# david8862/tf-keras-speech-commands

Hardware: AMD Instinct MI355X
Metric: 1 s@16 kHz clips/sec train-step, simple_cnn bs4096, 1/2/4/8 MI355X; eval top-1 (higher is better)
Workload: dtype f32; 1 GPU; configs[1]: simple_cnn train step = featurize(f32 1 s @16 kHz) + fwd + bwd + Adam, 36 logits (background + 35 words), batch 4096 per GPU; global_batch=4096, parallelism=dp1, gradient_exchange=none (one rank), rccl_ranks=0, library_build=546ca62dfe01

## Files before the change

### tf-keras-speech-commands_amd/csrc/kws_conv_group.h

```cpp
#pragma once

namespace kws {

constexpr int kGrThreads = 1024, kGrWaves = kGrThreads / 64;

template <int C, int G>
__device__ __forceinline__ void group_stats(float s, float ss, int ch, int grp, int lq, double *red, double *__restrict__ partial, int stride,
                                            double *__restrict__ acc = nullptr)
{
    double a = (double)s, q = (double)ss;
    a += __shfl_xor(a, 16, 64); a += __shfl_xor(a, 32, 64);
    q += __shfl_xor(q, 16, 64); q += __shfl_xor(q, 32, 64);
    if (lq == 0) { red[(grp * 2 + 0) * C + ch] = a; red[(grp * 2 + 1) * C + ch] = q; }
    __syncthreads();
    for (int i = threadIdx.x; i < 2 * C; i += kGrThreads) {
        const int which = i / C, n = i - which * C;
        double t = 0.0;
#pragma unroll
        for (int g2 = 0; g2 < G; ++g2) t += red[(g2 * 2 + which) * C + n];
        if (acc) acc_add(acc, 2 * C, i, t);
        else partial[((long)which * C + n) * stride + blockIdx.x] = t;
    }
}

// ... 139 lines not shown
        __shared__ __attribute__((aligned(16))) float cf3[2 * kFuC3];
        f32x4 sc, sh;
        if (g.in.acc) {
            bn_fwd_coef_prologue(g.in, kFuC3, cf3, cf3 + kFuC3);
            sc = *reinterpret_cast<const f32x4 *>(cf3 + 4 * (tid & 15)); sh = *reinterpret_cast<const f32x4 *>(cf3 + kFuC3 + 4 * (tid & 15));
        } else {
            sc = *reinterpret_cast<const f32x4 *>(g.sc3 + 4 * (tid & 15)); sh = *reinterpret_cast<const f32x4 *>(g.sh3 + 4 * (tid & 15));
        }
        for (int i = tid; i < kFuClips * PER; i += kGrThreads) {
            const int c = i / PER, r = i - c * PER, pos = r >> 4, u4 = r & 15;
            f32x4 v = {0.f, 0.f, 0.f, 0.f};
            if (b0 + c < g.B) {
                const f32x4 z = *reinterpret_cast<const f32x4 *>(g.z3 + ((long)(b0 + c) * PER + r) * 4);
#pragma unroll
                for (int e = 0; e < 4; ++e) v[e] = relu6f(fmaf(z[e], sc[e], sh[e]));
            }
            bf16x4 h, m, l;
            split_bf16(v, h, m, l);
            const int e0 = ((pos * kFuClips + c) * 8 + ((u4 >> 1) ^ ((c >> 1) & 7))) * 8 + (u4 & 1) * 4;
            *reinterpret_cast<bf16x4 *>(A3 + e0) = h;
            *reinterpret_cast<bf16x4 *>(A3 + kFuA3P + e0) = m;
            *reinterpret_cast<bf16x4 *>(A3 + 2 * kFuA3P + e0) = l;
        }
    }
    __syncthreads();
    f32x4 acc[NP];
#pragma unroll
    for (int q = 0; q < NP; ++q) acc[q] = (f32x4){0.f, 0.f, 0.f, 0.f};
#pragma unroll 1
    for (int ks3 = 0; ks3 < 18; ks3 += 3) {
#pragma unroll
        for (int d = 0; d < 3; ++d) {
            const int ks = ks3 + d;
            if (ks + 2 < 18) fu_load_b(g.f4, (long)(ks + 2) * 8 + ct, lane, b4[(d + 2) % 3]);
            const int tap = ks >> 1, chunk = ks & 1, kh = tap / 3, kw = tap - kh * 3;
            const int uo = ((4 * chunk + lq) ^ sw) * 8;
#pragma unroll
            for (int q = 0; q < NP; ++q) {
                const int pos = NP * grp + q, oh = pos / kFuW3, ow = pos - oh * kFuW3;
                const int ih = oh + kh - 1, iw = ow + kw - 1;
                if (ih >= 0 && ih < kFuH3 && iw >= 0 && iw < kFuW3) {
                    const __bf16 *row = A3 + ((ih * kFuW3 + iw) * kFuClips + li) * kFuC3 + uo;
                    bf16x8 a[3];
#pragma unroll
                    for (int p = 0; p < 3; ++p) a[p] = *reinterpret_cast<const bf16x8 *>(row + p * kFuA3P);
                    acc[q] = mfma_bf16x6(a, b4[d], acc[q]);
                }
            }
        }
    }
    const int ch = 16 * ct + li;
    float s = 0.f, ss = 0.f;
#pragma unroll
    for (int q = 0; q < NP; ++q) {
        const int pos = NP * grp + q;
#pragma unroll
        for (int r = 0; r < 4; ++r) {
            const int clip = 4 * lq + r;
            const float v = fmaxf(acc[q][r], 0.f);
            if (b0 + clip < g.B) g.z4[((long)(b0 + clip) * (kFuH3 * kFuW3) + pos) * kFuC4 + ch] = v;
            s += v; ss = fmaf(v, v, ss);
        }
    }
    __syncthreads();
    group_stats<kFuC4, kGrWaves / 8>(s, ss, ch, grp, lq, reinterpret_cast<double *>(gr_lds), g.partial, g.stride, g.acc);
}

constexpr int kGrD4P = kFuH3 * kFuW3 * kFuClips * kFuC4;
struct GroupDgrad4Args { const __bf16 *dz[3], *fw[3]; const float *z3, *coef; float *g3; double *partial; int stride, B; double *acc; };

__global__ __launch_bounds__(kGrThreads, 1) void conv4_group_dgrad_kernel(GroupDgrad4Args g)
{
    extern __shared__ __attribute__((aligned(16))) float gr_lds[];
    __bf16 *D4 = reinterpret_cast<__bf16 *>(gr_lds);
    const int tid = threadIdx.x, lane = tid & 63, wave = __builtin_amdgcn_readfirstlane(tid >> 6), li = lane & 15, lq = lane >> 4;
    const int b0 = blockIdx.x * kFuClips;
    constexpr int NP = 12 / (kGrWaves / 4);
    const int ct = wave & 3, grp = wave >> 2;
    bf16x8 bw[3][3];
    fu_load_b(g.fw, ct, lane, bw[0]);
    fu_load_b(g.fw, 4 + ct, lane, bw[1]);
    {
        constexpr int PER = kFuH3 * kFuW3 * kFuC4 / 8;
        for (int i = tid; i < 3 * kFuClips * PER; i += kGrThreads) {
            const int p = i / (kFuClips * PER), r0 = i - p * (kFuClips * PER), c = r0 / PER, r = r0 - c * PER, pos = r >> 4, u = r & 15;
            bf16x8 v = {0, 0, 0, 0, 0, 0, 0, 0};
            if (b0 + c < g.B) v = *reinterpret_cast<const bf16x8 *>(g.dz[p] + ((long)(b0 + c) * PER + r) * 8);
            *reinterpret_cast<bf16x8 *>(D4 + p * kGrD4P + ((pos * kFuClips + c) * 16 + (u ^ (c & 15))) * 8) = v;
        }
    }
    __syncthreads();
    f32x4 acc[NP];
#pragma unroll
    for (int q = 0; q < NP; ++q) acc[q] = (f32x4){0.f, 0.f, 0.f, 0.f};
#pragma unroll 1
    for (int ks3 = 0; ks3 < 36; ks3 += 3) {
#pragma unroll
        for (int d = 0; d < 3; ++d) {
            const int ks = ks3 + d;
            if (ks + 2 < 36) fu_load_b(g.fw, (long)(ks + 2) * 4 + ct, lane, bw[(d + 2) % 3]);
            const int tap = ks >> 2, chunk = ks & 3, kh = tap / 3, kw = tap - kh * 3;
            const int uo = ((4 * chunk + lq) ^ li) * 8;
#pragma unroll
            for (int q = 0; q < NP; ++q) {
                const int pos = NP * grp + q, y = pos / kFuW3, x = pos - y * kFuW3;
                const int sy = y + 1 - kh, sx = x + 1 - kw;
                if (sy >= 0 && sy < kFuH3 && sx >= 0 && sx < kFuW3) {
                    const __bf16 *row = D4 + ((sy * kFuW3 + sx) * kFuClips + li) * kFuC4 + uo;
                    bf16x8 a[3];
#pragma unroll
                    for (int p = 0; p < 3; ++p) a[p] = *reinterpret_cast<const bf16x8 *>(row + p * kGrD4P);
                    acc[q] = mfma_bf16x6(a, bw[d], acc[q]);
                }
            }
        }
    }
    const int ch = 16 * ct + li;
    const float gsc = g.coef[ch], gsh = g.coef[kFuC3 + ch], gmean = g.coef[2 * kFuC3 + ch], ginv = g.coef[3 * kFuC3 + ch];
    float s = 0.f, ss = 0.f;
    float z3v[NP][4];
#pragma unroll
    for (int q = 0; q < NP; ++q)
#pragma unroll
        for (int r = 0; r < 4; ++r) {
            const int clip = 4 * lq + r;
            z3v[q][r] = b0 + clip < g.B ? g.z3[((long)(b0 + clip) * (kFuH3 * kFuW3) + NP * grp + q) * kFuC3 + ch] : 0.f;
        }
#pragma unroll
    for (int q = 0; q < NP; ++q) {
        const int pos = NP * grp + q;
#pragma unroll
        for (int r = 0; r < 4; ++r) {
            const int clip = 4 * lq + r;
            if (b0 + clip < g.B) {
                const long e = ((long)(b0 + clip) * (kFuH3 * kFuW3) + pos) * kFuC3 + ch;
                const float zv = z3v[q][r], yv = fmaf(zv, gsc, gsh);
                const float v = (yv > 0.f && yv < 6.f) ? acc[q][r] : 0.f;
                g.g3[e] = v;
                s += v; ss = fmaf(v, (zv - gmean) * ginv, ss);
            }
        }
    }
    __syncthreads();
    group_stats<kFuC3, kGrWaves / 4>(s, ss, ch, grp, lq, reinterpret_cast<double *>(gr_lds), g.partial, g.stride, g.acc);
}

struct GroupDgrad3Args { const float *dz3; const __bf16 *fw[3]; float *da2; int B; const float *zmax2, *coef2; double *acc; };

__global__ __launch_bounds__(kGrThreads, 1) void conv3_group_dgrad_kernel(GroupDgrad3Args g)
{
    extern __shared__ __attribute__((aligned(16))) float gr_lds[];
    __bf16 *D3 = reinterpret_cast<__bf16 *>(gr_lds);
    const int tid = threadIdx.x, lane = tid & 63, wave = __builtin_amdgcn_readfirstlane(tid >> 6), li = lane & 15, lq = lane >> 4;
    const int b0 = blockIdx.x * kFuClips;
    const int sw = (li >> 1) & 7;
    constexpr int NPOS = kFuH2 * kFuW2, NG = kGrWaves / 2, NP = (NPOS + NG - 1) / NG;
    const int ct = wave & 1, grp = wave >> 1;
    bf16x8 bw[3][3];
    fu_load_b(g.fw, ct, lane, bw[0]);
    fu_load_b(g.fw, 2 + ct, lane, bw[1]);
    {
        constexpr int PER = kFuH3 * kFuW3 * kFuC3 / 4;
        for (int i = tid; i < kFuClips * PER; i += kGrThreads) {
            const int c = i / PER, r = i - c * PER, pos = r >> 4, u4 = r & 15;
            f32x4 v = {0.f, 0.f, 0.f, 0.f};
            if (b0 + c < g.B) v = *reinterpret_cast<const f32x4 *>(g.dz3 + ((long)(b0 + c) * PER + r) * 4);
            bf16x4 h, m, l;
            split_bf16(v, h, m, l);
            const int e0 = ((pos * kFuClips + c) * 8 + ((u4 >> 1) ^ ((c >> 1) & 7))) * 8 + (u4 & 1) * 4;
            *reinterpret_cast<bf16x4 *>(D3 + e0) = h;
            *reinterpret_cast<bf16x4 *>(D3 + kFuA3P + e0) = m;
            *reinterpret_cast<bf16x4 *>(D3 + 2 * kFuA3P + e0) = l;
        }
    }
    __syncthreads();
    f32x4 acc[NP];
#pragma unroll
    for (int q = 0; q < NP; ++q) acc[q] = (f32x4){0.f, 0.f, 0.f, 0.f};
#pragma unroll 1
    for (int ks3 = 0; ks3 < 18; ks3 += 3) {
#pragma unroll
        for (int d = 0; d < 3; ++d) {
            const int ks = ks3 + d;
            if (ks + 2 < 18) fu_load_b(g.fw, (long)(ks + 2) * 2 + ct, lane, bw[(d + 2) % 3]);
            const int tap = ks >> 1, chunk = ks & 1, kh = tap / 3, kw = tap - kh * 3;
            const int uo = ((4 * chunk + lq) ^ sw) * 8;
#pragma unroll
            for (int q = 0; q < NP; ++q) {
                const int pos = NP * grp + q, y = pos / kFuW2, x = pos - y * kFuW2;
                const int sy = y + 1 - kh, sx = x + 1 - kw;
                if (pos < NPOS && sy >= 0 && sx >= 0 && !((sy | sx) & 1) && (sy >> 1) < kFuH3 && (sx >> 1) < kFuW3) {
                    const __bf16 *row = D3 + (((sy >> 1) * kFuW3 + (sx >> 1)) * kFuClips + li) * kFuC3 + uo;
                    bf16x8 a[3];
#pragma unroll
                    for (int p = 0; p < 3; ++p) a[p] = *reinterpret_cast<const bf16x8 *>(row + p * kFuA3P);
                    acc[q] = mfma_bf16x6(a, bw[d], acc[q]);
                }
            }
        }
    }
    const int ch = 16 * ct + li;
    if (g.acc) {
        const float gsc = g.coef2[ch], gsh = g.coef2[kFuC2 + ch], gmean = g.coef2[2 * kFuC2 + ch], ginv = g.coef2[3 * kFuC2 + ch];
        float s = 0.f, sx = 0.f;
        float za[NP][4];
#pragma unroll
        for (int q = 0; q < NP; ++q)
#pragma unroll
            for (int r = 0; r < 4; ++r) {
                const int pos = NP * grp + q, clip = 4 * lq + r;
// ... 36 lines not shown
```

### tf-keras-speech-commands_amd/csrc/kws_dense_head.h

```cpp
#pragma once

namespace kws {

constexpr int kDhK = 128, kDhCP = 48, kDhCS = 50;
constexpr int kDhKS = kDhK + 8;

struct DenseHeadArgs {
    const float *a4;
    const __bf16 *fd[3], *fo[3];
    const float *db, *w2;
    float *d1, *dd1, *da4;
    float *dw2, *db2, *ddb;
    int B, C, flat;
    HeadFwdArgs fw;
    const float *zmax4 = nullptr, *coef4 = nullptr;
    double *acc4 = nullptr;
    float drop_rate = 0.f;
    uint32_t seed_lo = 0, seed_hi = 0;
    const float *z4 = nullptr;
    BnAccFwd in4{};
    float *a4w = nullptr, *zmax4w = nullptr;
    unsigned char *arg4w = nullptr;
    int H3 = 0, W3 = 0;
};

constexpr int kDhWaves = 8, kDhThreads = 64 * kDhWaves;
__global__ __launch_bounds__(kDhThreads) void dense_head_fused_kernel(DenseHeadArgs g)
{
    constexpr int NW = kDhWaves, NT = kDhThreads;
    static_assert(NW == 4 || NW == 8, "column tiles per wave below: 8 / NW Dense tiles, 24 / NW dW2 tiles");
    constexpr int DT = 8 / NW, WT = 24 / NW;
    extern __shared__ __attribute__((aligned(16))) float dh_lds[];
    const int RS4 = g.flat + 8;
    float *a4s = dh_lds;
    float *xs = a4s + 16 * RS4;
    float *dd = xs + 16 * kDhKS;
    float *ds = dd + 16 * kDhKS;
    float *ws = ds + 16 * kDhCS;
    const int tid = threadIdx.x, lane = tid & 63, wave = __builtin_amdgcn_readfirstlane(tid >> 6), li = lane & 15, lq = lane >> 4;
    const int b0 = blockIdx.x * 16, C = g.C, K = kDhK;
    const int nks = g.flat / 32;

    bf16x8 bcur[DT][3], bnext[DT][3];
#pragma unroll
    for (int t = 0; t < DT; ++t) fu_load_b(g.fd, DT * wave + t, lane, bcur[t]);
    constexpr int NW2 = kDhK * kDhCP / NT;
    static_assert(kDhK * kDhCP % NT == 0, "whole rounds");
    float w2v[NW2];
#pragma unroll
    for (int j = 0; j < NW2; ++j) { const int i = tid + j * NT, k = i / kDhCP, c = i - k * kDhCP; w2v[j] = c < C ? g.w2[(long)k * C + c] : 0.f; }
    __shared__ __attribute__((aligned(16))) float cf4[4 * kDhK];
    if (g.z4) {
        bn_fwd_coef_prologue(g.in4, kDhK, cf4, cf4 + kDhK, cf4 + 2 * kDhK, cf4 + 3 * kDhK);
        const int W4 = g.W3 / 2, nf4 = g.flat / 4;
        constexpr int NB = 2;
        for (int base = tid; base < 16 * nf4; base += NB * NT) {
            f32x4 z[NB][4];
#pragma unroll
            for (int k = 0; k < NB; ++k) {
                const int i = base + NT * k, r = i / nf4, u = i - r * nf4, win = u / (kDhK / 4), c0 = 4 * (u - win * (kDhK / 4));
                const int ph = win / W4, pw = win - ph * W4;
                const bool ok = i < 16 * nf4 && b0 + r < g.B;
                const float *zp = g.z4 + ((((long)(b0 + r) * g.H3 + 2 * ph) * g.W3 + 2 * pw) * kDhK + c0);
#pragma unroll
                for (int j = 0; j < 4; ++j)
                    z[k][j] = ok ? *reinterpret_cast<const f32x4 *>(zp + ((j >> 1) * g.W3 + (j & 1)) * kDhK) : (f32x4){0.f, 0.f, 0.f, 0.f};
            }
#pragma unroll
            for (int k = 0; k < NB; ++k) {
                const int i = base + NT * k, r = i / nf4, u = i - r * nf4, c0 = 4 * (u % (kDhK / 4));
                if (i >= 16 * nf4) continue;
                f32x4 v = {0.f, 0.f, 0.f, 0.f};
                if (b0 + r < g.B) {
                    const f32x4 sc = *reinterpret_cast<const f32x4 *>(cf4 + c0), sh = *reinterpret_cast<const f32x4 *>(cf4 + kDhK + c0);
                    const long o = (long)(b0 + r) * g.flat + 4 * u;
                    f32x4 zm;
                    unsigned am = 0u;
#pragma unroll
                    for (int e = 0; e < 4; ++e) {
                        const float y0 = fmaf(z[k][0][e], sc[e], sh[e]), y1 = fmaf(z[k][1][e], sc[e], sh[e]);
                        const float y2 = fmaf(z[k][2][e], sc[e], sh[e]), y3 = fmaf(z[k][3][e], sc[e], sh[e]);
                        float a = relu6f(fmaxf(fmaxf(y0, y1), fmaxf(y2, y3)));
                        unsigned arg = 0u;
                        float best = relu6f(y0), zz = z[k][0][e];
                        const float v1 = relu6f(y1), v2 = relu6f(y2), v3 = relu6f(y3);
                        if (v1 > best) { best = v1; arg = 1u; zz = z[k][1][e]; }
                        if (v2 > best) { best = v2; arg = 2u; zz = z[k][2][e]; }
                        if (v3 > best) { arg = 3u; zz = z[k][3][e]; }
                        zm[e] = zz;
                        am |= arg << (8 * e);
                        if (g.drop_rate > 0.f) a = dropout_keep(g.seed_lo, g.seed_hi, (uint32_t)(o + e), g.drop_rate) ? a / (1.f - g.drop_rate) : 0.f;
                        v[e] = a;
                    }
                    *reinterpret_cast<f32x4 *>(g.a4w + o) = v;
                    *reinterpret_cast<f32x4 *>(g.zmax4w + o) = zm;
                    *reinterpret_cast<unsigned *>(g.arg4w + o) = am;
                }
                *reinterpret_cast<f32x4 *>(a4s + r * RS4 + 4 * u) = v;
            }
        }
    } else
    for (int i = tid; i < 16 * (g.flat / 4); i += NT) {
        const int r = i / (g.flat / 4), u = i - r * (g.flat / 4);
        f32x4 v = {0.f, 0.f, 0.f, 0.f};
        if (b0 + r < g.B) v = *reinterpret_cast<const f32x4 *>(g.a4 + (long)(b0 + r) * g.flat + 4 * u);
        *reinterpret_cast<f32x4 *>(a4s + r * RS4 + 4 * u) = v;
    }
#pragma unroll
    for (int j = 0; j < NW2; ++j) { const int i = tid + j * NT, k = i / kDhCP, c = i - k * kDhCP; ws[k * kDhCS + c] = w2v[j]; }
    __syncthreads();

    {
        f32x4 acc[DT];
#pragma unroll
        for (int t = 0; t < DT; ++t) acc[t] = (f32x4){0.f, 0.f, 0.f, 0.f};
        for (int ks = 0; ks < nks; ++ks) {
            if (ks + 1 < nks)
#pragma unroll
                for (int t = 0; t < DT; ++t) fu_load_b(g.fd, (long)(ks + 1) * 8 + DT * wave + t, lane, bnext[t]);
            bf16x8 a[3];
            fu_load_a(a4s + li * RS4 + 32 * ks + 4 * lq, a);
#pragma unroll
            for (int t = 0; t < DT; ++t) acc[t] = mfma_bf16x6(a, bcur[t], acc[t]);
#pragma unroll
            for (int t = 0; t < DT; ++t)
#pragma unroll
                for (int p = 0; p < 3; ++p) bcur[t][p] = bnext[t][p];
        }
#pragma unroll
        for (int t = 0; t < DT; ++t) {
            const int ch = 16 * (DT * wave + t) + li;
            const float bias = g.db[ch];
#pragma unroll
            for (int r = 0; r < 4; ++r) {
                const float v = relu6f(acc[t][r] + bias);
                xs[(4 * lq + r) * kDhKS + ch] = v;
                if (g.d1 && b0 + 4 * lq + r < g.B) g.d1[(long)(b0 + 4 * lq + r) * K + ch] = v;
            }
        }
    }
    const int nct = g.flat / 16, tpw = nct / NW;
    __syncthreads();

    const HeadFwdArgs &fw = g.fw;
    {
        const int sm = (tid >> 4) & 15, j = tid & 15, b = b0 + sm;
        const bool has = tid < 256;
        float *lg = ds + sm * kDhCS;
        if (wave < kDhCP / 16) {
            f32x4 acc = {0.f, 0.f, 0.f, 0.f};
            for (int kk = 0; kk < K / 4; ++kk) acc = mfma16(xs[li * kDhKS + 4 * kk + lq], ws[(4 * kk + lq) * kDhCS + 16 * wave + li], acc);
            const int cc = 16 * wave + li;
            const float bv = cc < C ? fw.b2[cc] : 0.f;
#pragma unroll
            for (int r = 0; r < 4; ++r) ds[(4 * lq + r) * kDhCS + cc] = acc[r] + bv;
        }
        __syncthreads();
        if (has) {
        float mx = -INFINITY;
        int am = 0x7fffffff;
        for (int c = j; c < C; c += 16) {
            const float v = lg[c];
            if (v > mx) { mx = v; am = c; }
        }
#pragma unroll
        for (int o = 8; o > 0; o >>= 1) {
            const float omx = __shfl_xor(mx, o, 16);
            const int oam = __shfl_xor(am, o, 16);
            if (omx > mx || (omx == mx && oam < am)) { mx = omx; am = oam; }
        }
        float sum = 0.f;
        for (int c = j; c < C; c += 16) { const float e = expf(lg[c] - mx); lg[c] = e; sum += e; }
#pragma unroll
        for (int o = 8; o > 0; o >>= 1) sum += __shfl_xor(sum, o, 16);
        const float rs = 1.f / sum;
        const bool live = b < g.B;
        const int y = live ? fw.labels[b] : 0;
        const float py = lg[y] * rs;
        float loss, coef;
        if (fw.class_w) {
            loss = -logf(py) * fw.class_w[y];
            coef = fw.class_w[y];
        } else {
            const float lo = kCeEps, hi = 1.f - kCeEps;
            loss = -logf(fminf(fmaxf(py, lo), hi));
            coef = (py >= lo && py <= hi) ? 1.f : 0.f;
        }
        if (fw.ignore_index > 0 && y == fw.ignore_index) { loss = 0.f; coef = 0.f; }
        if (live && j == 0) { fw.loss_i_out[b] = loss; fw.correct_i_out[b] = am == y ? 1.f : 0.f; }
        if (live && fw.probs)
            for (int c = j; c < C; c += 16) fw.probs[(long)b * C + c] = lg[c] * rs;
        for (int c = j; c < kDhCP; c += 16)
            lg[c] = (live && c < C) ? (lg[c] * rs - (c == y ? 1.f : 0.f)) * coef * fw.grad_scale : 0.f;
        }
    }
    __syncthreads();

    f32x4 accw[WT];
#pragma unroll
    for (int q = 0; q < WT; ++q) accw[q] = (f32x4){0.f, 0.f, 0.f, 0.f};
    for (int nt = wave; nt < K / 16; nt += NW) {
        f32x4 acc = {0.f, 0.f, 0.f, 0.f};
#pragma unroll
        for (int j = 0; j < kDhCP / 4; ++j) acc = mfma16(ds[li * kDhCS + 4 * j + lq], ws[(16 * nt + li) * kDhCS + 4 * j + lq], acc);
        float cs = 0.f;
#pragma unroll
        for (int r = 0; r < 4; ++r) {
            const int row = 4 * lq + r, k = 16 * nt + li;
            const float xv = xs[row * kDhKS + k];
            float v = (xv > 0.f && xv < 6.f) ? acc[r] : 0.f;
            if (b0 + row >= g.B) v = 0.f;
            dd[row * kDhKS + k] = v;
            if (b0 + row < g.B) g.dd1[(long)(b0 + row) * K + k] = v;
            cs += v;
        }
        cs += __shfl_xor(cs, 16, 64);
        cs += __shfl_xor(cs, 32, 64);
        if (lq == 0) atomicAdd(g.ddb + 16 * nt + li, cs);
    }
#pragma unroll
    for (int q = 0; q < WT; ++q) {
        const int t = wave + NW * q, mt = t / 3, nt = t - 3 * mt;
#pragma unroll
        for (int j = 0; j < 4; ++j) accw[q] = mfma16(xs[(4 * j + lq) * kDhKS + 16 * mt + li], ds[(4 * j + lq) * kDhCS + 16 * nt + li], accw[q]);
    }
    float accb = 0.f;
    if (tid < C)
        for (int r = 0; r < 16; ++r) accb += ds[r * kDhCS + tid];
    __syncthreads();

    {
        bf16x8 a[4][3];
#pragma unroll
        for (int kk = 0; kk < 4; ++kk) {
            const float *row = dd + li * kDhKS + 32 * kk + 8 * lq;
            fu_split(*reinterpret_cast<const f32x4 *>(row), *reinterpret_cast<const f32x4 *>(row + 4), a[kk]);
        }
        float za[4] = {0.f, 0.f, 0.f, 0.f}, zan[4] = {0.f, 0.f, 0.f, 0.f};
        if (g.acc4)
#pragma unroll
            for (int r = 0; r < 4; ++r)
                if (b0 + 4 * lq + r < g.B) za[r] = g.zmax4[(long)(b0 + 4 * lq + r) * g.flat + 16 * wave + li];
        for (int i = 0; i < tpw; ++i) {
            const int nt = wave + NW * i, tap = nt / (kDhK / 16), ctl = nt - tap * (kDhK / 16);
            f32x4 acc = {0.f, 0.f, 0.f, 0.f};
            bf16x8 b[4][3];
#pragma unroll
            for (int kk = 0; kk < 4; ++kk) fu_load_b(g.fo, (long)(tap * 4 + kk) * (kDhK / 16) + ctl, lane, b[kk]);
            if (g.acc4 && i + 1 < tpw)
#pragma unroll
                for (int r = 0; r < 4; ++r)
                    if (b0 + 4 * lq + r < g.B) zan[r] = g.zmax4[(long)(b0 + 4 * lq + r) * g.flat + 16 * (nt + NW) + li];
#pragma unroll
            for (int kk = 0; kk < 4; ++kk) acc = mfma_bf16x6(a[kk], b[kk], acc);
            if (g.acc4) {
                const int ch = 16 * ctl + li;
                const float *cf = g.z4 ? cf4 : g.coef4;
                const float gsc = cf[ch], gsh = cf[kDhK + ch], gmean = cf[2 * kDhK + ch], ginv = cf[3 * kDhK + ch];
                float s = 0.f, sx = 0.f;
#pragma unroll
                for (int r = 0; r < 4; ++r)
                    if (b0 + 4 * lq + r < g.B) {
                        const long e = (long)(b0 + 4 * lq + r) * g.flat + 16 * nt + li;
                        float v = acc[r];
                        if (g.drop_rate > 0.f) v = dropout_keep(g.seed_lo, g.seed_hi, (uint32_t)e, g.drop_rate) ? v / (1.f - g.drop_rate) : 0.f;
                        const float ya = fmaf(za[r], gsc, gsh);
                        v = (ya > 0.f && ya < 6.f) ? v : 0.f;
                        g.da4[e] = v;
                        s += v; sx = fmaf(v, (za[r] - gmean) * ginv, sx);
                    }
                double sd = (double)s, sxd = (double)sx;
                sd += __shfl_xor(sd, 16, 64); sd += __shfl_xor(sd, 32, 64);
                sxd += __shfl_xor(sxd, 16, 64); sxd += __shfl_xor(sxd, 32, 64);
                if (lq == 0) { acc_add(g.acc4, 2 * kDhK, ch, sd); acc_add(g.acc4, 2 * kDhK, kDhK + ch, sxd); }
#pragma unroll
                for (int r = 0; r < 4; ++r) za[r] = zan[r];
            } else {
#pragma unroll
                for (int r = 0; r < 4; ++r)
                    if (b0 + 4 * lq + r < g.B) g.da4[(long)(b0 + 4 * lq + r) * g.flat + 16 * nt + li] = acc[r];
            }
        }
    }
#pragma unroll
    for (int q = 0; q < WT; ++q) {
        const int t = wave + NW * q, mt = t / 3, nt = t - 3 * mt, c = 16 * nt + li;
        if (c < C) {
#pragma unroll
            for (int r = 0; r < 4; ++r) ws[(16 * mt + 4 * lq + r) * C + c] = accw[q][r];
        }
    }
    __syncthreads();
    for (int i = tid; i < K * C; i += NT) atomicAdd(g.dw2 + i, ws[i]);
    if (tid < C) atomicAdd(g.db2 + tid, accb);
}

}
```

### tf-keras-speech-commands_amd/csrc/kws_layers.h

```cpp
#pragma once
#include "kws_device.h"

namespace kws {

constexpr float kBnEps = 1e-3f;
constexpr double kBnMomentum = 0.99;
constexpr float kCeEps = 1e-7f;
constexpr int kStatStride = 1024;

__device__ __forceinline__ double block_sum_partials(const double *__restrict__ partial, int which, int C, int c, int nblk,
                                                     double *sh )
{
    double s = 0.0;
    for (int b = threadIdx.x; b < nblk; b += 256) s += partial[((long)which * C + c) * kStatStride + b];
    sh[threadIdx.x] = s;
    __syncthreads();
    for (int o = 128; o > 0; o >>= 1) {
        if ((int)threadIdx.x < o) sh[threadIdx.x] += sh[threadIdx.x + o];
        __syncthreads();
    }
    s = sh[0];
    __syncthreads();
    return s;
}

__device__ __forceinline__ double wave_sum_partials(const double *__restrict__ partial, int which, int C, int c, int nblk)
{
    const double *p = partial + ((long)which * C + c) * kStatStride;
    const int lane = threadIdx.x & 63;
    double v[kStatStride / 64];
#pragma unroll
    for (int j = 0; j < kStatStride / 64; ++j) v[j] = lane + 64 * j < nblk ? p[lane + 64 * j] : 0.0;
    double s = 0.0;
#pragma unroll
    for (int j = 0; j < kStatStride / 64; ++j) s += v[j];
#pragma unroll
    for (int o = 32; o > 0; o >>= 1) s += __shfl_xor(s, o, 64);
    return s;
}

__global__ __launch_bounds__(256) void channel_stats_kernel(const float *__restrict__ z, long M, int C, int rows_per_block,
                                                             double *__restrict__ partial)
{
    const int c = threadIdx.x % C, r = threadIdx.x / C, R = 256 / C;
    const long beg = (long)blockIdx.x * rows_per_block;
    const long end = beg + rows_per_block < M ? beg + rows_per_block : M;
    double s = 0.0, ss = 0.0;
    for (long m = beg + r; m < end; m += 4 * R) {
        float v[4];
#pragma unroll
        for (int u = 0; u < 4; ++u) { const long mm = m + (long)u * R; v[u] = z[(mm < end ? mm : end - 1) * C + c]; }
#pragma unroll
        for (int u = 0; u < 4; ++u) {
            const double x = m + (long)u * R < end ? (double)v[u] : 0.0;
            s += x;
            ss += x * x;
        }
    }
    __shared__ double sh[2][256];
    sh[0][threadIdx.x] = s;
    sh[1][threadIdx.x] = ss;
    __syncthreads();
    if (r == 0) {
        for (int j = 1; j < R; ++j) { s += sh[0][j * C + c]; ss += sh[1][j * C + c]; }
        partial[((long)0 * C + c) * kStatStride + blockIdx.x] = s;
        partial[((long)1 * C + c) * kStatStride + blockIdx.x] = ss;
    }
}

struct BnCoef {
    float *scale, *shift, *mean, *inv, *k2, *k3;
};

__global__ void bn_finalize_train_kernel(const double *__restrict__ partial, int nblk, long M, int C,
                                         const float *__restrict__ gamma, const float *__restrict__ beta,
                                         float *__restrict__ moving_mean, float *__restrict__ moving_var, BnCoef k)
{
    const int c = blockIdx.x;
    const double s = wave_sum_partials(partial, 0, C, c, nblk);
    const double ss = wave_sum_partials(partial, 1, C, c, nblk);
    if (threadIdx.x != 0) return;
    const double mean = s / (double)M;
    double var = ss / (double)M - mean * mean;
    var = var < 0.0 ? 0.0 : var;
    const double inv = 1.0 / sqrt(var + (double)kBnEps);
    const double sc = (double)gamma[c] * inv;
    k.scale[c] = (float)sc;
    k.shift[c] = (float)((double)beta[c] - mean * sc);
    k.mean[c] = (float)mean;
    k.inv[c] = (float)inv;
    const double unbiased = var * ((double)M / (double)(M > 1 ? M - 1 : 1));
    moving_mean[c] = (float)((double)moving_mean[c] * kBnMomentum + mean * (1.0 - kBnMomentum));
    moving_var[c] = (float)((double)moving_var[c] * kBnMomentum + unbiased * (1.0 - kBnMomentum));
}

struct BnAccFwd { const double *acc; double *acc_clear_set; long M; const float *gamma, *beta; float *moving_mean, *moving_var; BnCoef k; };
__device__ __forceinline__ void bn_fwd_coef_prologue(const BnAccFwd &a, int C, float *sc, float *sh, float *mean_out = nullptr, float *inv_out = nullptr)
{
    const int c = threadIdx.x;
    if (c < C) {
        const double s = acc_sum(a.acc, 2 * C, c), ss = acc_sum(a.acc, 2 * C, C + c);
        const double mean = s / (double)a.M;
        double var = ss / (double)a.M - mean * mean;
        var = var < 0.0 ? 0.0 : var;
        const double inv = 1.0 / sqrt(var + (double)kBnEps);
        const double scd = (double)a.gamma[c] * inv;
        const float scf = (float)scd, shf = (float)((double)a.beta[c] - mean * scd);
        sc[c] = scf;
        sh[c] = shf;
        if (mean_out) { mean_out[c] = (float)mean; inv_out[c] = (float)inv; }
        if (blockIdx.x == 0) {
            a.k.scale[c] = scf;
            a.k.shift[c] = shf;
            a.k.mean[c] = (float)mean;
            a.k.inv[c] = (float)inv;
            const double unbiased = var * ((double)a.M / (double)(a.M > 1 ? a.M - 1 : 1));
            a.moving_mean[c] = (float)((double)a.moving_mean[c] * kBnMomentum + mean * (1.0 - kBnMomentum));
            a.moving_var[c] = (float)((double)a.moving_var[c] * kBnMomentum + unbiased * (1.0 - kBnMomentum));
        }
    }
    if (blockIdx.x == 0 && a.acc_clear_set) acc_clear(a.acc_clear_set, threadIdx.x, blockDim.x);
    __syncthreads();
}

__global__ void bn_infer_coef_kernel(int C, const float *__restrict__ gamma, const float *__restrict__ beta,
                                     const float *__restrict__ moving_mean, const float *__restrict__ moving_var, BnCoef k)
{
    const int c = blockIdx.x * blockDim.x + threadIdx.x;
    if (c >= C) return;
    const double inv = 1.0 / sqrt((double)moving_var[c] + (double)kBnEps);
    const double sc = (double)gamma[c] * inv;
    k.scale[c] = (float)sc;
    k.shift[c] = (float)((double)beta[c] - (double)moving_mean[c] * sc);
    k.mean[c] = moving_mean[c];
    k.inv[c] = (float)inv;
}

struct BnInferAll { int C[4]; const float *gamma[4], *beta[4], *mm[4], *mv[4]; BnCoef k[4]; };
__global__ void bn_infer_coef_all_kernel(BnInferAll a)
{
    const int l = blockIdx.x, c = threadIdx.x;
    if (c >= a.C[l]) return;
    const double inv = 1.0 / sqrt((double)a.mv[l][c] + (double)kBnEps);
    const double sc = (double)a.gamma[l][c] * inv;
    a.k[l].scale[c] = (float)sc;
    a.k[l].shift[c] = (float)((double)a.beta[l][c] - (double)a.mm[l][c] * sc);
    a.k[l].mean[c] = a.mm[l][c];
    a.k[l].inv[c] = (float)inv;
}

template <bool POOL>
__global__ __launch_bounds__(256) void bn_act_pool_kernel(const float *__restrict__ z, const float *__restrict__ scale,
                                                           const float *__restrict__ shift, float *__restrict__ a, int B,
                                                           int H, int W, int C, float drop_rate, uint32_t seed_lo,
                                                           uint32_t seed_hi, float *__restrict__ zmax_out = nullptr,
                                                           unsigned char *__restrict__ arg_out = nullptr)
{
    const int Hp = POOL ? H / 2 : H, Wp = POOL ? W / 2 : W;
    const long total = (long)B * Hp * Wp * C, idx = (long)blockIdx.x * 256 + threadIdx.x;
    if (idx >= total) return;
    const int c = (int)(idx % C);
    long t = idx / C;
    const int pw = (int)(t % Wp);
    t /= Wp;
    const int ph = (int)(t % Hp), b = (int)(t / Hp);
    const float sc = scale[c], sh = shift[c];
    float v;
    if (POOL) {
        const float *p = z + (((long)b * H + 2 * ph) * W + 2 * pw) * C + c;
        const float z0 = p[0], z1 = p[C], z2 = p[(long)W * C], z3 = p[(long)W * C + C];
        const float y0 = fmaf(z0, sc, sh), y1 = fmaf(z1, sc, sh), y2 = fmaf(z2, sc, sh), y3 = fmaf(z3, sc, sh);
        v = fmaxf(fmaxf(y0, y1), fmaxf(y2, y3));
        if (zmax_out) {
            int arg = 0;
            float best = relu6f(y0), zm = z0;
            const float v1 = relu6f(y1), v2 = relu6f(y2), v3 = relu6f(y3);
            if (v1 > best) { best = v1; arg = 1; zm = z1; }
            if (v2 > best) { best = v2; arg = 2; zm = z2; }
            if (v3 > best) { arg = 3; zm = z3; }
            zmax_out[idx] = zm;
            arg_out[idx] = (unsigned char)arg;
        }
    } else {
        v = fmaf(z[idx], sc, sh);
    }
    v = relu6f(v);
    if (drop_rate > 0.f) v = dropout_keep(seed_lo, seed_hi, (uint32_t)idx, drop_rate) ? v / (1.f - drop_rate) : 0.f;
    a[idx] = v;
}

__global__ __launch_bounds__(256) void bn_act_pool_acc_kernel(const float *__restrict__ z, BnAccFwd in, float *__restrict__ a, int B, int H, int W,
                                                               int C, float drop_rate, uint32_t seed_lo, uint32_t seed_hi,
                                                               float *__restrict__ zmax_out, unsigned char *__restrict__ arg_out)
{
    __shared__ float cf[256];
    bn_fwd_coef_prologue(in, C, cf, cf + 128);
    const int Hp = H / 2, Wp = W / 2;
    const long total = (long)B * Hp * Wp * C;
    for (long idx = (long)blockIdx.x * 256 + threadIdx.x; idx < total; idx += (long)gridDim.x * 256) {
        const int c = (int)(idx % C);
        long t = idx / C;
        const int pw = (int)(t % Wp);
        t /= Wp;
        const int ph = (int)(t % Hp), b = (int)(t / Hp);
        const float sc = cf[c], sh = cf[128 + c];
// ... 868 lines not shown
```

Measured before the change: 7.890 million clips/s.

## Hoist global loads ahead of dependent work in dense head and group dgrad

In the conv4 group dgrad kernel, the staging loop now issues all global loads before any LDS store. The z3 and coefficient loads move ahead of the MFMA loop so their latency overlaps compute. In the dense head kernel, BN coefficient reads are split into an issue step and a finish step that overlap the first z4 tile load. The Dense-product weight fragments use a 4-deep register ring, and scalar loads (bias, labels, class weights, dgrad fragments, zmax) are hoisted early. This adds register pressure, and a waves_per_eu hint is set to balance occupancy, which could cause spills.

```diff
diff --git a/tf-keras-speech-commands_amd/csrc/kws_conv_group.h b/tf-keras-speech-commands_amd/csrc/kws_conv_group.h
--- a/tf-keras-speech-commands_amd/csrc/kws_conv_group.h
+++ b/tf-keras-speech-commands_amd/csrc/kws_conv_group.h
@@ -245,14 +245,32 @@
     fu_load_b(g.fw, 4 + ct, lane, bw[1]);
     {
         constexpr int PER = kFuH3 * kFuW3 * kFuC4 / 8;
-        for (int i = tid; i < 3 * kFuClips * PER; i += kGrThreads) {
-            const int p = i / (kFuClips * PER), r0 = i - p * (kFuClips * PER), c = r0 / PER, r = r0 - c * PER, pos = r >> 4, u = r & 15;
-            bf16x8 v = {0, 0, 0, 0, 0, 0, 0, 0};
-            if (b0 + c < g.B) v = *reinterpret_cast<const bf16x8 *>(g.dz[p] + ((long)(b0 + c) * PER + r) * 8);
-            *reinterpret_cast<bf16x8 *>(D4 + p * kGrD4P + ((pos * kFuClips + c) * 16 + (u ^ (c & 15))) * 8) = v;
-        }
-    }
-    __syncthreads();
+        constexpr int NIT = 3 * kFuClips * PER / kGrThreads;
+        static_assert(3 * kFuClips * PER % kGrThreads == 0, "whole rounds");
+        bf16x8 v[NIT];
+#pragma unroll
+        for (int k = 0; k < NIT; ++k) {
+            const int i = tid + k * kGrThreads, p = i / (kFuClips * PER), r0 = i - p * (kFuClips * PER), c = r0 / PER, r = r0 - c * PER;
+            v[k] = (bf16x8){0, 0, 0, 0, 0, 0, 0, 0};
+            if (b0 + c < g.B) v[k] = *reinterpret_cast<const bf16x8 *>(g.dz[p] + ((long)(b0 + c) * PER + r) * 8);
+        }
+#pragma unroll
+        for (int k = 0; k < NIT; ++k) {
+            const int i = tid + k * kGrThreads, p = i / (kFuClips * PER), r0 = i - p * (kFuClips * PER), c = r0 / PER, r = r0 - c * PER, pos = r >> 4, u = r & 15;
+            *reinterpret_cast<bf16x8 *>(D4 + p * kGrD4P + ((pos * kFuClips + c) * 16 + (u ^ (c & 15))) * 8) = v[k];
+        }
+    }
+    __syncthreads();
+    const int ch = 16 * ct + li;
+    const float gsc = g.coef[ch], gsh = g.coef[kFuC3 + ch], gmean = g.coef[2 * kFuC3 + ch], ginv = g.coef[3 * kFuC3 + ch];
+    float z3v[NP][4];
+#pragma unroll
+    for (int q = 0; q < NP; ++q)
+#pragma unroll
+        for (int r = 0; r < 4; ++r) {
+            const int clip = 4 * lq + r;
+            z3v[q][r] = b0 + clip < g.B ? g.z3[((long)(b0 + clip) * (kFuH3 * kFuW3) + NP * grp + q) * kFuC3 + ch] : 0.f;
+        }
     f32x4 acc[NP];
 #pragma unroll
     for (int q = 0; q < NP; ++q) acc[q] = (f32x4){0.f, 0.f, 0.f, 0.f};
@@ -278,17 +296,7 @@
             }
         }
     }
-    const int ch = 16 * ct + li;
-    const float gsc = g.coef[ch], gsh = g.coef[kFuC3 + ch], gmean = g.coef[2 * kFuC3 + ch], ginv = g.coef[3 * kFuC3 + ch];
     float s = 0.f, ss = 0.f;
-    float z3v[NP][4];
-#pragma unroll
-    for (int q = 0; q < NP; ++q)
-#pragma unroll
-        for (int r = 0; r < 4; ++r) {
-            const int clip = 4 * lq + r;
-            z3v[q][r] = b0 + clip < g.B ? g.z3[((long)(b0 + clip) * (kFuH3 * kFuW3) + NP * grp + q) * kFuC3 + ch] : 0.f;
-        }
 #pragma unroll
     for (int q = 0; q < NP; ++q) {
         const int pos = NP * grp + q;
diff --git a/tf-keras-speech-commands_amd/csrc/kws_dense_head.h b/tf-keras-speech-commands_amd/csrc/kws_dense_head.h
--- a/tf-keras-speech-commands_amd/csrc/kws_dense_head.h
+++ b/tf-keras-speech-commands_amd/csrc/kws_dense_head.h
@@ -25,7 +25,9 @@
 };
 
 constexpr int kDhWaves = 8, kDhThreads = 64 * kDhWaves;
-__global__ __launch_bounds__(kDhThreads) void dense_head_fused_kernel(DenseHeadArgs g)
+constexpr int kDhRing = 4;
+static_assert(kDhK % (32 * kDhRing) == 0, "the Dense product consumes whole rings");
+__global__ __launch_bounds__(kDhThreads) __attribute__((amdgpu_waves_per_eu(3))) void dense_head_fused_kernel(DenseHeadArgs g)
 {
     constexpr int NW = kDhWaves, NT = kDhThreads;
     static_assert(NW == 4 || NW == 8, "column tiles per wave below: 8 / NW Dense tiles, 24 / NW dW2 tiles");
@@ -41,63 +43,93 @@
     const int b0 = blockIdx.x * 16, C = g.C, K = kDhK;
     const int nks = g.flat / 32;
 
-    bf16x8 bcur[DT][3], bnext[DT][3];
-#pragma unroll
-    for (int t = 0; t < DT; ++t) fu_load_b(g.fd, DT * wave + t, lane, bcur[t]);
+    __shared__ __attribute__((aligned(16))) float cf4[4 * kDhK];
+    const int W4 = g.W3 / 2, nf4 = g.flat / 4;
+    constexpr int NB = 2;
+    const auto load = [&](int base, f32x4 (&z)[NB][4]) {
+#pragma unroll
+        for (int k = 0; k < NB; ++k) {
+            const int i = base + NT * k, r = i / nf4, u = i - r * nf4, win = u / (kDhK / 4), c0 = 4 * (u - win * (kDhK / 4));
+            const int ph = win / W4, pw = win - ph * W4;
+            const bool ok = i < 16 * nf4 && b0 + r < g.B;
+            const float *zp = g.z4 + ((((long)(b0 + r) * g.H3 + 2 * ph) * g.W3 + 2 * pw) * kDhK + c0);
+#pragma unroll
+            for (int j = 0; j < 4; ++j)
+                z[k][j] = ok ? *reinterpret_cast<const f32x4 *>(zp + ((j >> 1) * g.W3 + (j & 1)) * kDhK) : (f32x4){0.f, 0.f, 0.f, 0.f};
+        }
+    };
+    const auto finish = [&](int base, const f32x4 (&z)[NB][4]) {
+#pragma unroll
+        for (int k = 0; k < NB; ++k) {
+            const int i = base + NT * k, r = i / nf4, u = i - r * nf4, c0 = 4 * (u % (kDhK / 4));
+            if (i >= 16 * nf4) continue;
+            f32x4 v = {0.f, 0.f, 0.f, 0.f};
+            if (b0 + r < g.B) {
+                const f32x4 sc = *reinterpret_cast<const f32x4 *>(cf4 + c0), sh = *reinterpret_cast<const f32x4 *>(cf4 + kDhK + c0);
+                const long o = (long)(b0 + r) * g.flat + 4 * u;
+                f32x4 zm;
+                unsigned am = 0u;
+#pragma unroll
+                for (int e = 0; e < 4; ++e) {
+                    const float y0 = fmaf(z[k][0][e], sc[e], sh[e]), y1 = fmaf(z[k][1][e], sc[e], sh[e]);
+                    const float y2 = fmaf(z[k][2][e], sc[e], sh[e]), y3 = fmaf(z[k][3][e], sc[e], sh[e]);
+                    float a = relu6f(fmaxf(fmaxf(y0, y1), fmaxf(y2, y3)));
+                    unsigned arg = 0u;
+                    float best = relu6f(y0), zz = z[k][0][e];
+                    const float v1 = relu6f(y1), v2 = relu6f(y2), v3 = relu6f(y3);
+                    if (v1 > best) { best = v1; arg = 1u; zz = z[k][1][e]; }
+                    if (v2 > best) { best = v2; arg = 2u; zz = z[k][2][e]; }
+                    if (v3 > best) { arg = 3u; zz = z[k][3][e]; }
+                    zm[e] = zz;
+                    am |= arg << (8 * e);
+                    if (g.drop_rate > 0.f) a = dropout_keep(g.seed_lo, g.seed_hi, (uint32_t)(o + e), g.drop_rate) ? a / (1.f - g.drop_rate) : 0.f;
+                    v[e] = a;
+                }
+                *reinterpret_cast<f32x4 *>(g.a4w + o) = v;
+                *reinterpret_cast<f32x4 *>(g.zmax4w + o) = zm;
+                *reinterpret_cast<unsigned *>(g.arg4w + o) = am;
+            }
+            *reinterpret_cast<f32x4 *>(a4s + r * RS4 + 4 * u) = v;
+        }
+    };
+    f32x4 z0[NB][4];
+    if (g.z4) {
+        BnFwdCoefRegs cr;
+        bn_fwd_coef_issue(g.in4, kDhK, cr);
+        load(tid, z0);
+        bn_fwd_coef_finish(g.in4, kDhK, cr, cf4, cf4 + kDhK, cf4 + 2 * kDhK, cf4 + 3 * kDhK);
+    }
+    constexpr int NR = kDhRing;
+    bf16x8 br[NR][DT][3];
+#pragma unroll
+    for (int q = 0; q < NR / 2; ++q)
+#pragma unroll
+        for (int t = 0; t < DT; ++t) fu_load_b(g.fd, (long)q * 8 + DT * wave + t, lane, br[q][t]);
     constexpr int NW2 = kDhK * kDhCP / NT;
     static_assert(kDhK * kDhCP % NT == 0, "whole rounds");
     float w2v[NW2];
 #pragma unroll
     for (int j = 0; j < NW2; ++j) { const int i = tid + j * NT, k = i / kDhCP, c = i - k * kDhCP; w2v[j] = c < C ? g.w2[(long)k * C + c] : 0.f; }
-    __shared__ __attribute__((aligned(16))) float cf4[4 * kDhK];
+    const HeadFwdArgs &fw = g.fw;
+    float dbv[DT];
+#pragma unroll
+    for (int t = 0; t < DT; ++t) dbv[t] = g.db[16 * (DT * wave + t) + li];
+    const float b2v = (wave < kDhCP / 16 && 16 * wave + li < C) ? fw.b2[16 * wave + li] : 0.f;
+    const bool hlive = tid < 256 && b0 + ((tid >> 4) & 15) < g.B;
+    const int hy = hlive ? fw.labels[b0 + ((tid >> 4) & 15)] : 0;
+    const float hcw = (hlive && fw.class_w) ? fw.class_w[hy] : 0.f;
+    if (g.z4) finish(tid, z0);
+#pragma unroll
+    for (int j = 0; j < NW2; ++j) { const int i = tid + j * NT, k = i / kDhCP, c = i - k * kDhCP; ws[k * kDhCS + c] = w2v[j]; }
+#pragma unroll
+    for (int q = NR / 2; q < NR; ++q)
+#pragma unroll
+        for (int t = 0; t < DT; ++t) fu_load_b(g.fd, (long)q * 8 + DT * wave + t, lane, br[q][t]);
     if (g.z4) {
-        bn_fwd_coef_prologue(g.in4, kDhK, cf4, cf4 + kDhK, cf4 + 2 * kDhK, cf4 + 3 * kDhK);
-        const int W4 = g.W3 / 2, nf4 = g.flat / 4;
-        constexpr int NB = 2;
-        for (int base = tid; base < 16 * nf4; base += NB * NT) {
+        for (int base = tid + NB * NT; base < 16 * nf4; base += NB * NT) {
             f32x4 z[NB][4];
-#pragma unroll
-            for (int k = 0; k < NB; ++k) {
-                const int i = base + NT * k, r = i / nf4, u = i - r * nf4, win = u / (kDhK / 4), c0 = 4 * (u - win * (kDhK / 4));
-                const int ph = win / W4, pw = win - ph * W4;
-                const bool ok = i < 16 * nf4 && b0 + r < g.B;
-                const float *zp = g.z4 + ((((long)(b0 + r) * g.H3 + 2 * ph) * g.W3 + 2 * pw) * kDhK + c0);
-#pragma unroll
-                for (int j = 0; j < 4; ++j)
-                    z[k][j] = ok ? *reinterpret_cast<const f32x4 *>(zp + ((j >> 1) * g.W3 + (j & 1)) * kDhK) : (f32x4){0.f, 0.f, 0.f, 0.f};
-            }
-#pragma unroll
-            for (int k = 0; k < NB; ++k) {
-                const int i = base + NT * k, r = i / nf4, u = i - r * nf4, c0 = 4 * (u % (kDhK / 4));
-                if (i >= 16 * nf4) continue;
-                f32x4 v = {0.f, 0.f, 0.f, 0.f};
-                if (b0 + r < g.B) {
-                    const f32x4 sc = *reinterpret_cast<const f32x4 *>(cf4 + c0), sh = *reinterpret_cast<const f32x4 *>(cf4 + kDhK + c0);
-                    const long o = (long)(b0 + r) * g.flat + 4 * u;
-                    f32x4 zm;
-                    unsigned am = 0u;
-#pragma unroll
-                    for (int e = 0; e < 4; ++e) {
-                        const float y0 = fmaf(z[k][0][e], sc[e], sh[e]), y1 = fmaf(z[k][1][e], sc[e], sh[e]);
-                        const float y2 = fmaf(z[k][2][e], sc[e], sh[e]), y3 = fmaf(z[k][3][e], sc[e], sh[e]);
-                        float a = relu6f(fmaxf(fmaxf(y0, y1), fmaxf(y2, y3)));
-                        unsigned arg = 0u;
-                        float best = relu6f(y0), zz = z[k][0][e];
-                        const float v1 = relu6f(y1), v2 = relu6f(y2), v3 = relu6f(y3);
-                        if (v1 > best) { best = v1; arg = 1u; zz = z[k][1][e]; }
-                        if (v2 > best) { best = v2; arg = 2u; zz = z[k][2][e]; }
-                        if (v3 > best) { arg = 3u; zz = z[k][3][e]; }
-                        zm[e] = zz;
-                        am |= arg << (8 * e);
-                        if (g.drop_rate > 0.f) a = dropout_keep(g.seed_lo, g.seed_hi, (uint32_t)(o + e), g.drop_rate) ? a / (1.f - g.drop_rate) : 0.f;
-                        v[e] = a;
-                    }
-                    *reinterpret_cast<f32x4 *>(g.a4w + o) = v;
-                    *reinterpret_cast<f32x4 *>(g.zmax4w + o) = zm;
-                    *reinterpret_cast<unsigned *>(g.arg4w + o) = am;
-                }
-                *reinterpret_cast<f32x4 *>(a4s + r * RS4 + 4 * u) = v;
-            }
+            load(base, z);
+            finish(base, z);
         }
     } else
     for (int i = tid; i < 16 * (g.flat / 4); i += NT) {
@@ -106,31 +138,30 @@
         if (b0 + r < g.B) v = *reinterpret_cast<const f32x4 *>(g.a4 + (long)(b0 + r) * g.flat + 4 * u);
         *reinterpret_cast<f32x4 *>(a4s + r * RS4 + 4 * u) = v;
     }
-#pragma unroll
-    for (int j = 0; j < NW2; ++j) { const int i = tid + j * NT, k = i / kDhCP, c = i - k * kDhCP; ws[k * kDhCS + c] = w2v[j]; }
     __syncthreads();
 
     {
         f32x4 acc[DT];
 #pragma unroll
         for (int t = 0; t < DT; ++t) acc[t] = (f32x4){0.f, 0.f, 0.f, 0.f};
-        for (int ks = 0; ks < nks; ++ks) {
-            if (ks + 1 < nks)
-#pragma unroll
-                for (int t = 0; t < DT; ++t) fu_load_b(g.fd, (long)(ks + 1) * 8 + DT * wave + t, lane, bnext[t]);
-            bf16x8 a[3];
-            fu_load_a(a4s + li * RS4 + 32 * ks + 4 * lq, a);
-#pragma unroll
-            for (int t = 0; t < DT; ++t) acc[t] = mfma_bf16x6(a, bcur[t], acc[t]);
-#pragma unroll
-            for (int t = 0; t < DT; ++t)
-#pragma unroll
-                for (int p = 0; p < 3; ++p) bcur[t][p] = bnext[t][p];
+#pragma unroll 1
+        for (int ks0 = 0; ks0 < nks; ks0 += NR) {
+#pragma unroll
+            for (int q = 0; q < NR; ++q) {
+                const int ks = ks0 + q;
+                bf16x8 a[3];
+                fu_load_a(a4s + li * RS4 + 32 * ks + 4 * lq, a);
+#pragma unroll
+                for (int t = 0; t < DT; ++t) acc[t] = mfma_bf16x6(a, br[q][t], acc[t]);
+                if (ks + NR < nks)
+#pragma unroll
+                    for (int t = 0; t < DT; ++t) fu_load_b(g.fd, (long)(ks + NR) * 8 + DT * wave + t, lane, br[q][t]);
+            }
         }
 #pragma unroll
         for (int t = 0; t < DT; ++t) {
             const int ch = 16 * (DT * wave + t) + li;
-            const float bias = g.db[ch];
+            const float bias = dbv[t];
 #pragma unroll
             for (int r = 0; r < 4; ++r) {
                 const float v = relu6f(acc[t][r] + bias);
@@ -142,7 +173,6 @@
     const int nct = g.flat / 16, tpw = nct / NW;
     __syncthreads();
 
-    const HeadFwdArgs &fw = g.fw;
     {
         const int sm = (tid >> 4) & 15, j = tid & 15, b = b0 + sm;
         const bool has = tid < 256;
@@ -151,9 +181,8 @@
             f32x4 acc = {0.f, 0.f, 0.f, 0.f};
             for (int kk = 0; kk < K / 4; ++kk) acc = mfma16(xs[li * kDhKS + 4 * kk + lq], ws[(4 * kk + lq) * kDhCS + 16 * wave + li], acc);
             const int cc = 16 * wave + li;
-            const float bv = cc < C ? fw.b2[cc] : 0.f;
-#pragma unroll
-            for (int r = 0; r < 4; ++r) ds[(4 * lq + r) * kDhCS + cc] = acc[r] + bv;
+#pragma unroll
+            for (int r = 0; r < 4; ++r) ds[(4 * lq + r) * kDhCS + cc] = acc[r] + b2v;
         }
         __syncthreads();
         if (has) {
@@ -175,12 +204,12 @@
         for (int o = 8; o > 0; o >>= 1) sum += __shfl_xor(sum, o, 16);
         const float rs = 1.f / sum;
         const bool live = b < g.B;
-        const int y = live ? fw.labels[b] : 0;
+        const int y = hy;
         const float py = lg[y] * rs;
         float loss, coef;
         if (fw.class_w) {
-            loss = -logf(py) * fw.class_w[y];
-            coef = fw.class_w[y];
+            loss = -logf(py) * hcw;
+            coef = hcw;
         } else {
             const float lo = kCeEps, hi = 1.f - kCeEps;
             loss = -logf(fminf(fmaxf(py, lo), hi));
@@ -193,6 +222,19 @@
         for (int c = j; c < kDhCP; c += 16)
             lg[c] = (live && c < C) ? (lg[c] * rs - (c == y ? 1.f : 0.f)) * coef * fw.grad_scale : 0.f;
         }
+    }
+    const auto dg_frag = [&](int nt, int kk) { return (long)(nt / (kDhK / 16) * 4 + kk) * (kDhK / 16) + nt % (kDhK / 16); };
+    const auto dg_zmax = [&](int nt, float (&z)[4]) {
+#pragma unroll
+        for (int r = 0; r < 4; ++r) z[r] = b0 + 4 * lq + r < g.B ? g.zmax4[(long)(b0 + 4 * lq + r) * g.flat + 16 * nt + li] : 0.f;
+    };
+    bf16x8 bg[4][3];
+#pragma unroll
+    for (int kk = 0; kk < 4; ++kk) fu_load_b(g.fo, dg_frag(wave, kk), lane, bg[kk]);
+    float za[4] = {0.f, 0.f, 0.f, 0.f}, zan[4] = {0.f, 0.f, 0.f, 0.f};
+    if (g.acc4) {
+        dg_zmax(wave, za);
+        if (tpw > 1) dg_zmax(wave + NW, zan);
     }
     __syncthreads();
 
@@ -229,30 +271,29 @@
         for (int r = 0; r < 16; ++r) accb += ds[r * kDhCS + tid];
     __syncthreads();
 
+#pragma unroll
+    for (int q = 0; q < WT; ++q) {
+        const int t = wave + NW * q, mt = t / 3, nt = t - 3 * mt, c = 16 * nt + li;
+        if (c < C) {
+#pragma unroll
+            for (int r = 0; r < 4; ++r) ws[(16 * mt + 4 * lq + r) * C + c] = accw[q][r];
+        }
+    }
+
     {
-        bf16x8 a[4][3];
-#pragma unroll
-        for (int kk = 0; kk < 4; ++kk) {
-            const float *row = dd + li * kDhKS + 32 * kk + 8 * lq;
-            fu_split(*reinterpret_cast<const f32x4 *>(row), *reinterpret_cast<const f32x4 *>(row + 4), a[kk]);
-        }
-        float za[4] = {0.f, 0.f, 0.f, 0.f}, zan[4] = {0.f, 0.f, 0.f, 0.f};
-        if (g.acc4)
-#pragma unroll
-            for (int r = 0; r < 4; ++r)
-                if (b0 + 4 * lq + r < g.B) za[r] = g.zmax4[(long)(b0 + 4 * lq + r) * g.flat + 16 * wave + li];
         for (int i = 0; i < tpw; ++i) {
-            const int nt = wave + NW * i, tap = nt / (kDhK / 16), ctl = nt - tap * (kDhK / 16);
+            const int nt = wave + NW * i, ctl = nt % (kDhK / 16);
             f32x4 acc = {0.f, 0.f, 0.f, 0.f};
-            bf16x8 b[4][3];
-#pragma unroll
-            for (int kk = 0; kk < 4; ++kk) fu_load_b(g.fo, (long)(tap * 4 + kk) * (kDhK / 16) + ctl, lane, b[kk]);
-            if (g.acc4 && i + 1 < tpw)
-#pragma unroll
-                for (int r = 0; r < 4; ++r)
-                    if (b0 + 4 * lq + r < g.B) zan[r] = g.zmax4[(long)(b0 + 4 * lq + r) * g.flat + 16 * (nt + NW) + li];
-#pragma unroll
-            for (int kk = 0; kk < 4; ++kk) acc = mfma_bf16x6(a[kk], b[kk], acc);
+            float zann[4] = {0.f, 0.f, 0.f, 0.f};
+            if (g.acc4 && i + 2 < tpw) dg_zmax(nt + 2 * NW, zann);
+#pragma unroll
+            for (int kk = 0; kk < 4; ++kk) {
+                const float *row = dd + li * kDhKS + 32 * kk + 8 * lq;
+                bf16x8 a[3];
+                fu_split(*reinterpret_cast<const f32x4 *>(row), *reinterpret_cast<const f32x4 *>(row + 4), a);
+                acc = mfma_bf16x6(a, bg[kk], acc);
+                if (i + 1 < tpw) fu_load_b(g.fo, dg_frag(nt + NW, kk), lane, bg[kk]);
+            }
             if (g.acc4) {
                 const int ch = 16 * ctl + li;
                 const float *cf = g.z4 ? cf4 : g.coef4;
@@ -274,20 +315,12 @@
                 sxd += __shfl_xor(sxd, 16, 64); sxd += __shfl_xor(sxd, 32, 64);
                 if (lq == 0) { acc_add(g.acc4, 2 * kDhK, ch, sd); acc_add(g.acc4, 2 * kDhK, kDhK + ch, sxd); }
 #pragma unroll
-                for (int r = 0; r < 4; ++r) za[r] = zan[r];
+                for (int r = 0; r < 4; ++r) { za[r] = zan[r]; zan[r] = zann[r]; }
             } else {
 #pragma unroll
                 for (int r = 0; r < 4; ++r)
                     if (b0 + 4 * lq + r < g.B) g.da4[(long)(b0 + 4 * lq + r) * g.flat + 16 * nt + li] = acc[r];
             }
-        }
-    }
-#pragma unroll
-    for (int q = 0; q < WT; ++q) {
-        const int t = wave + NW * q, mt = t / 3, nt = t - 3 * mt, c = 16 * nt + li;
-        if (c < C) {
-#pragma unroll
-            for (int r = 0; r < 4; ++r) ws[(16 * mt + 4 * lq + r) * C + c] = accw[q][r];
         }
     }
     __syncthreads();
diff --git a/tf-keras-speech-commands_amd/csrc/kws_layers.h b/tf-keras-speech-commands_amd/csrc/kws_layers.h
--- a/tf-keras-speech-commands_amd/csrc/kws_layers.h
+++ b/tf-keras-speech-commands_amd/csrc/kws_layers.h
@@ -95,17 +95,33 @@
 }
 
 struct BnAccFwd { const double *acc; double *acc_clear_set; long M; const float *gamma, *beta; float *moving_mean, *moving_var; BnCoef k; };
-__device__ __forceinline__ void bn_fwd_coef_prologue(const BnAccFwd &a, int C, float *sc, float *sh, float *mean_out = nullptr, float *inv_out = nullptr)
+struct BnFwdCoefRegs { double s[kAccSlots], ss[kAccSlots]; float gamma, beta; };
+__device__ __forceinline__ void bn_fwd_coef_issue(const BnAccFwd &a, int C, BnFwdCoefRegs &r)
 {
     const int c = threadIdx.x;
     if (c < C) {
-        const double s = acc_sum(a.acc, 2 * C, c), ss = acc_sum(a.acc, 2 * C, C + c);
+#pragma unroll
+        for (int j = 0; j < kAccSlots; ++j) { r.s[j] = a.acc[j * 2 * C + c]; r.ss[j] = a.acc[j * 2 * C + C + c]; }
+        r.gamma = a.gamma[c];
+        r.beta = a.beta[c];
+    }
+}
+__device__ __forceinline__ void bn_fwd_coef_finish(const BnAccFwd &a, int C, const BnFwdCoefRegs &r, float *sc, float *sh, float *mean_out = nullptr,
+                                                   float *inv_out = nullptr)
+{
+    const int c = threadIdx.x;
+    if (c < C) {
+        double s = 0.0, ss = 0.0;
+#pragma unroll
+        for (int j = 0; j < kAccSlots; ++j) s += r.s[j];
+#pragma unroll
+        for (int j = 0; j < kAccSlots; ++j) ss += r.ss[j];
         const double mean = s / (double)a.M;
         double var = ss / (double)a.M - mean * mean;
         var = var < 0.0 ? 0.0 : var;
         const double inv = 1.0 / sqrt(var + (double)kBnEps);
-        const double scd = (double)a.gamma[c] * inv;
-        const float scf = (float)scd, shf = (float)((double)a.beta[c] - mean * scd);
+        const double scd = (double)r.gamma * inv;
+        const float scf = (float)scd, shf = (float)((double)r.beta - mean * scd);
         sc[c] = scf;
         sh[c] = shf;
         if (mean_out) { mean_out[c] = (float)mean; inv_out[c] = (float)inv; }
@@ -121,6 +137,12 @@
     }
     if (blockIdx.x == 0 && a.acc_clear_set) acc_clear(a.acc_clear_set, threadIdx.x, blockDim.x);
     __syncthreads();
+}
+__device__ __forceinline__ void bn_fwd_coef_prologue(const BnAccFwd &a, int C, float *sc, float *sh, float *mean_out = nullptr, float *inv_out = nullptr)
+{
+    BnFwdCoefRegs r;
+    bn_fwd_coef_issue(a, C, r);
+    bn_fwd_coef_finish(a, C, r, sc, sh, mean_out, inv_out);
 }
 
 __global__ void bn_infer_coef_kernel(int C, const float *__restrict__ gamma, const float *__restrict__ beta,
```

New measurement: 7.911 million clips/s, median of 3. Within noise of the previous version (+0.3%).
